# yuxng/PoseCNN

Measured on AMD Instinct MI355X. Metric: RGB-D frames/sec (640x480, 21 classes), higher is better.
Workload: dtype f32

## Files before the change

### __graft_entry__.py

```python
import glob
import os
import subprocess
import sys

ROOT = os.path.dirname(os.path.abspath(__file__))
if ROOT not in sys.path:
    sys.path.insert(0, ROOT)


def build():
    env = dict(os.environ)
    env.setdefault("PYTORCH_ROCM_ARCH", "gfx950")
    jobs = str(min(8, os.cpu_count() or 1))
    subprocess.check_call(["make", "-C", os.path.join(ROOT, "posecnn_amd", "csrc"), "-j", jobs], env=env)
    subprocess.check_call(["make", "-C", os.path.join(ROOT, "oracle")], env=env)
    subprocess.check_call(["make", "-C", os.path.join(ROOT, "oracle"), "ref"], env=env)
    headers = sorted(glob.glob(os.path.join(ROOT, "include", "*.h"))) + sorted(glob.glob(os.path.join(ROOT, "include", "*", "*.h")))
    subprocess.check_call(["gcc", "-std=c11", "-Wall", "-Wextra", "-Werror", "-I" + os.path.join(ROOT, "include")] +
                          [arg for h in headers for arg in ("-include", h)] +
                          [os.path.join(ROOT, "tests", "capi_consumer.c"), "-o", os.path.join(ROOT, "tests", "capi_consumer"),
                           "-L" + os.path.join(ROOT, "posecnn_amd"), "-lposecnn_hip",
                           "-Wl,-rpath,$ORIGIN/../posecnn_amd", "-Wl,-rpath-link,/opt/rocm/lib"], env=env)
    import posecnn_amd
    from posecnn_amd import _lib
    _lib.lib()


def smoke():
    import numpy as np
    import torch

    sys.path.insert(0, os.path.join(ROOT, "tests"))
    import oracle
    from posecnn_amd import config, ops, synth

    assert torch.cuda.is_available(), "smoke() needs a GPU"
    dev = torch.device("cuda:0")
    K = config.DEMO_INTRINSICS.copy()
    K[:2] *= 320 / 640.0
    label, vertex, _ = synth.make_batch(100, 2, H=240, W=320, C=22, n_obj=3, K=K)
    meta = np.stack([config.make_meta_data(K)] * 2)
    ext = config.LOV_EXTENTS
    want = oracle.hough_voting(label, vertex, ext, meta, None, 0, -1.0, 0.02, 10, label_thr=200, padded=True)

    L = torch.from_numpy
    got = ops.hough_voting_gpu_padded(L(label).to(dev), L(vertex).to(dev), L(ext).to(dev), L(meta).to(dev),
                                      None, 0, -1.0, 0.02, 10, label_threshold=200)
    torch.cuda.synchronize()
    names = ("top_box", "top_pose", "top_target", "top_weight", "top_domain", "num_rois")
    for name, g, w in zip(names, got, want):
        g = g.cpu().numpy()
        assert np.array_equal(g.view(np.uint32), np.ascontiguousarray(w).view(np.uint32)), "smoke: %s differs from the oracle" % name
    assert int(got[5][1]) >= 2, "smoke: expected detections"

    rng = np.random.default_rng(0)
    feat = rng.standard_normal((2, 15, 20, 512)).astype(np.float32)
    r = int(want[5][0])
    top, arg = ops.roi_pool(L(feat).to(dev), got[0][:r].contiguous(), 7, 7, 1.0 / 16, 0)
    wt, wa = oracle.roi_pool(feat, want[0][:r], 7, 7, 1.0 / 16, 0)
    assert np.array_equal(top.cpu().numpy(), wt) and np.array_equal(arg.cpu().numpy(), wa), "smoke: roi_pool differs"
    print("smoke ok: %d detections, hough + roi_pool bit-identical to the oracle" % int(got[5][1]))


if __name__ == "__main__":
    build()
    if len(sys.argv) > 1 and sys.argv[1] == "smoke":
        smoke()
```

### posecnn_amd/_lib.py

```python
import ctypes
import glob
import os
import re
from ctypes import (POINTER, c_char_p, c_float, c_int, c_int64, c_long, c_size_t, c_uint32, c_uint64, c_void_p)

_HERE = os.path.dirname(os.path.abspath(__file__))
LIB_PATH = os.path.join(_HERE, "libposecnn_hip.so")

PCNN_OK = 0
PCNN_EINVAL = -1
PCNN_EWORKSPACE = -2
PCNN_EHIP = -3
PCNN_ENULL = -4

MAX_ROI = 128
HOUGH_ROWS_CAPACITY = MAX_ROI * 9
VERTEX_CHANNELS = 3
POSE_CHANNELS = 4

INCLUDE_DIR = os.path.join(os.path.dirname(_HERE), "include")

_RESTYPES = {"int": c_int, "long": c_long, "uint32_t": c_uint32, "const char*": c_char_p}
_SCALARS = {"int": c_int, "long": c_long, "float": c_float, "size_t": c_size_t, "int64_t": c_int64, "uint32_t": c_uint32,
            "uint64_t": c_uint64}
# ... 19 lines not shown
            raise ValueError("%s: not `type* [name]`" % where)
        return _POINTERS.get(" ".join(base), c_void_p)
    base = " ".join(tokens[:-1] if len(tokens) > 1 else tokens)
    if base not in _SCALARS:
        raise ValueError("%s: scalar type '%s' is not one of %s" % (where, base, sorted(_SCALARS)))
    return _SCALARS[base]


def parse_header(header, text):
    text = re.sub(r"^[ \t]*#.*$", "", _strip_comments(text), flags=re.M)
    found = {}
    for m in re.finditer(r"\b(pcnn_\w+)\s*\(", text):
        name, depth, end = m.group(1), 1, m.end()
        while depth and end < len(text):
            depth += {"(": 1, ")": -1}.get(text[end], 0)
            end += 1
        if depth or not re.match(r"\s*;", text[end:]):
            raise ValueError("%s: %s: not a prototype `ret %s(params);`" % (header, name, name))
        ret = re.sub(r"\s*\*\s*", "*", " ".join(re.split(r"[;{}]", text[:m.start()])[-1].split()))
        if ret not in _RESTYPES:
            raise ValueError("%s: %s: return type '%s' is not one of %s" % (header, name, ret, sorted(_RESTYPES)))
        if name in found:
            raise ValueError("%s: %s is declared twice" % (header, name))
        params, depth = [""], 0
        for ch in text[m.end():end - 1]:
            depth += {"(": 1, "[": 1, ")": -1, "]": -1}.get(ch, 0)
            if ch == "," and not depth:
                params.append("")
            else:
                params[-1] += ch
        params = [" ".join(p.split()) for p in params]
        found[name] = (_RESTYPES[ret], [] if params == ["void"] else
                       [_argtype(p, "%s: %s: parameter %d '%s'" % (header, name, i + 1, p)) for i, p in enumerate(params)])
    return found


def parse_headers(texts):
    out, owner = {}, {}
    for header, text in texts:
        out[header] = parse_header(header, text)
        for name in out[header]:
            if name in owner:
                raise ValueError("%s: %s is already declared in %s" % (header, name, owner[name]))
            owner[name] = header
    return out


def header_texts():
    top = sorted(glob.glob(os.path.join(INCLUDE_DIR, "*.h")))
    sub = sorted(glob.glob(os.path.join(INCLUDE_DIR, "*", "*.h")))
    return [(os.path.relpath(p, INCLUDE_DIR).replace(os.sep, "/"), open(p).read()) for p in top + sub]


def header_abi_version(texts=None):
    text = dict(header_texts() if texts is None else texts)["posecnn_hip.h"]
    return int(re.search(r"^[ \t]*#[ \t]*define[ \t]+PCNN_ABI_VERSION[ \t]+(\d+)[ \t]*$", _strip_comments(text), flags=re.M).group(1))


def profile_enable(on=True):
    call("pcnn_profile_enable", 1 if on else 0)


def profile_report(reset=True):
    import json
    L = lib()
    n = L.pcnn_profile_report(None, 0)
    buf = ctypes.create_string_buffer(int(n) + 16)
    L.pcnn_profile_report(buf, len(buf))
    if reset:
        L.pcnn_profile_reset()
    rep = json.loads(buf.value.decode())
    return {k.strip("()"): v for k, v in rep.items()}

_lib = None


class PoseCNNHipError(RuntimeError):

    def __init__(self, fn, status, message):
        super().__init__("%s failed: status %d (%s)" % (fn, status, message))
        self.status = status


def lib():
    global _lib
    if _lib is None:
        if not os.path.exists(LIB_PATH):
            raise RuntimeError(
                "libposecnn_hip.so not found at %s — build it with "
                "`python -c 'import __graft_entry__ as g; g.build()'` or "
                "`make -C posecnn_amd/csrc`. There is no CPU/PyTorch fallback." % LIB_PATH)
        import torch
        handle = ctypes.CDLL(LIB_PATH)
        texts = header_texts()
        bindings = parse_headers(texts)
        for table in bindings.values():
            for name, (res, args) in table.items():
                fn = getattr(handle, name)
                fn.restype = res
                fn.argtypes = args
        if handle.pcnn_abi_version() != header_abi_version(texts):
            raise RuntimeError("libposecnn_hip.so ABI version mismatch")
        BINDINGS.update(bindings)
        _lib = handle
    return _lib


def check(fn_name, status):
    if status != PCNN_OK:
        msg = lib().pcnn_last_error_string()
        msg = msg.decode("utf-8", "replace") if msg else ""
        if status in (PCNN_EINVAL, PCNN_ENULL):
            raise ValueError("%s: %s" % (fn_name, msg))
        raise PoseCNNHipError(fn_name, status, msg)


def call(name, *args):
    check(name, getattr(lib(), name)(*args))
```

### posecnn_amd/networks.py

```python
import math
import os

import numpy as np
import torch
import torch.nn.functional as F

from . import ops, pipeline

DEFAULT_PADDING = "SAME"


def layer(op):

    def layer_decorated(self, *args, **kwargs):
        name = kwargs.setdefault("name", self.get_unique_name(op.__name__))
        if len(self.inputs) == 0:
            raise RuntimeError("No input variables found for layer %s." % name)
        elif len(self.inputs) == 1:
            layer_input = self.inputs[0]
        else:
            layer_input = list(self.inputs)
        if isinstance(layer_input, list):
            layer_input = [i.activate(self) if isinstance(i, _Pending) else i for i in layer_input]
        elif (isinstance(layer_input, _Pending) and op.__name__ != "max_pool"
# ... 79 lines not shown

    def _pool2(self, net):
        return None


class _PendingFirst(_Pending):
    def __init__(self, x, w, bias, relu):
        _Pending.__init__(self, tuple(x.shape[:3]) + (w.shape[3],), bias, relu)
        self.x, self.w = x, w

    def _activate(self, net):
        return net._conv_first(raw_frame_blob(self.x), self.w.permute(3, 2, 0, 1), self.bias, self.relu)

    def frames(self):
        return (self.x if self.x.dtype == torch.uint8 else None, self.x if self.x.dtype == torch.uint16 else None)

    def next_v(self):
        if _is_raw(self.x):
            return ops.conv3x3_c3_winograd43_raw(*self.frames(), self.w, self.bias, self.relu)
        return ops.conv3x3_c3_winograd43(self.x, self.w, self.bias, self.relu)


class _PendingConv12(_Pending):
    def __init__(self, pf, name, w, bias, relu):
        _Pending.__init__(self, pf.shape[:3] + (w.shape[0],), bias, relu)
        self.pf, self.name, self.w = pf, name, w

    def _activate(self, net):
        ut, pk = net._winograd_bank(self.name, self.w)
        return ops.winograd43_conv(self.pf.next_v(), ut, self.bias, *self.shape[:3], self.relu, pool=0, packed=pk)

    def _pool2(self, net):
        pf = self.pf
        frag = net._derived(("conv12_frag", self.name), (self.w,),
                            lambda: ops.conv12_fragment_major(net._winograd_filter(self.name, self.w, transposed=True)),
                            net.winograd_tile)
        if _is_raw(pf.x):
            return ops.conv1_1_conv1_2_fused_raw(*pf.frames(), pf.w, pf.bias, frag, self.bias, pf.relu, self.relu, ut2_layout=1)
        return ops.conv1_1_conv1_2_fused(pf.x, pf.w, pf.bias, frag, self.bias, pf.relu, self.relu, groups=1, ut2_layout=1)


class _PendingGemm(_Pending):
    def __init__(self, v, ut, B, H, W, packed, bias, relu):
        _Pending.__init__(self, (B, H, W, ut.shape[-2]), bias, relu)
        self.v, self.ut, self.packed = v, ut, packed

    def _activate(self, net, pool=0):
        return ops.winograd43_conv(self.v, self.ut, self.bias, *self.shape[:3], self.relu, pool=pool, packed=self.packed)

    def _pool2(self, net):
        return self._activate(net, pool=1)


class _PendingWino(_Pending):
    def __init__(self, m, B, H, W, tile, dual, bias, relu):
        _Pending.__init__(self, (B, H, W, m.shape[2]), bias, relu)
        self.m, self.tile, self.dual = m, tile, dual

    def _activate(self, net, pool=False):
        return ops.winograd_output(self.m, self.bias, *self.shape[:3], self.relu, pool=pool, tile=self.tile)

    def _pool2(self, net):
        if not self.dual:
            return self._activate(net, pool=True)
        self.out, pooled = ops.winograd43_output_both(self.m, self.bias, *self.shape[:3], self.relu)
        return pooled


class _PendingBias(_Pending):
    def __init__(self, y, bias, relu, train=None):
        _Pending.__init__(self, tuple(y.shape), bias, relu)
        self.y, self.train = y, train

    def _activate(self, net):
        return net._bias_act(self.y, self.bias, self.relu)

    def _pool2(self, net):
        if self.train is not None:
            return _nhwc(ops.bias_relu_pool2_train(self.train, self.bias, self.relu))
        return net._bias_relu_pool2(self.y, self.bias, self.relu)


class _ConvAndPool(_Pending):
    def __init__(self, out, pooled, bias, relu):
        _Pending.__init__(self, tuple(out.shape), bias, relu, out, pooled)


class Network(object):

    fused_train_epilogue = False

    def use_fused_train_epilogue(self, on=True):
        self.fused_train_epilogue = bool(on)
        return self

    winograd_packed = True

    def __init__(self, device="cuda", seed=3, init="he", trainable=True):
        self.inputs = []
        self.layers = {}
        self.vars = {}
        self.device = torch.device(device)
        self.trainable = trainable
        self.init = init
        self._gen = torch.Generator(device="cpu").manual_seed(seed)
        self.keep_prob_queue = 1.0
        self.conv_timing = None
        self.winograd_min_channels = 64
        self.winograd_tile = 4
        self._cache = {}
        self.winograd_mfma = True
        self.fuse_first_conv_into_winograd = True
        self.fused_first_conv = True
        self.fused_conv12 = True
        self.defer_act = frozenset()
        self.dual_pool = frozenset()
        self.rows_count = None
        self.fc_skinny = True
        self.small_heads = True
        self.small_heads_max_pixels = 2 * 60 * 80

    def setup(self):
        raise NotImplementedError("Must be subclassed.")

    def feed(self, *args):
        assert len(args) != 0
        self.inputs = []
        for l in args:
            if isinstance(l, str):
                l = self.get_output(l)
            self.inputs.append(l)
        return self

    def get_output(self, name):
        try:
            out = self.layers[name]
        except KeyError:
            raise KeyError("Unknown layer name fed: %s" % name)
        if isinstance(out, _Lazy):
            out = self.layers[name] = out.fn()
        if isinstance(out, _Pending):
            out = self.layers[name] = out.activate(self)
        return out

    def _conv12_fused_at(self, H, W):
        return self.fused_conv12 and self.winograd_mfma and H % 16 == 0 and W % 16 == 0

    def _winograd_filter(self, name, w, transposed=False):
        def build():
            u = ops.winograd_filter(w, self.winograd_tile)
            return u.transpose(1, 2).contiguous() if transposed else u
        return self._derived(("wino", name, transposed), (w,), build, self.winograd_tile)

    def _winograd_bank(self, name, w):
        if not self.winograd_packed:
            return self._winograd_filter(name, w, transposed=True), False
        return self._derived(("wino_packed", name), (w,),
                             lambda: ops.winograd43_pack_filters(self._winograd_filter(name, w, transposed=True)),
                             self.winograd_tile), True

    def _derived(self, slot, sources, build, extra=None):
        hit = self._cache.get(slot)
        if hit is not None and hit[2] == extra and len(hit[0]) == len(sources):
            held, versions = hit[0], hit[1]
            i = 0
            for s in sources:
                if s is not held[i] or s._version != versions[i]:
                    break
                i += 1
            else:
                return hit[3]
        value = build()
        self._cache[slot] = (tuple(sources), tuple(s._version for s in sources), extra, value)
        return value

    def _timing(self, extra):
        if self.conv_timing is not None:
            timing = (torch.cuda.Event(enable_timing=True), torch.cuda.Event(enable_timing=True), extra)
            timing[0].record()
            return timing

    def _timed(self, name, timing, executed, direct):
        if timing is not None:
            timing[1].record()
            self.conv_timing.append((name, executed + timing[2], direct + timing[2], timing[0], timing[1]))

    def _conv_winograd(self, name, input, w, b, relu, c_i, c_o, tile):
        B_, H_, W_ = input.shape[:3]
        first = isinstance(input, _PendingFirst)
        timing = self._timing(2.0 * B_ * H_ * W_ * c_i * 27 if first else 0.0)
        v = input.next_v() if first else ops.winograd_input(input, tile)
        if tile == 4 and self.winograd_mfma and c_i % 64 == 0 and c_o % 64 == 0:
            ut, pk = self._winograd_bank(name, w)
            self._timed(name, timing, 0.0, 0.0)
            even = H_ % 2 == 0 and W_ % 2 == 0
            if name in self.defer_act and even:
                return _PendingGemm(v, ut, B_, H_, W_, pk, b, relu)
            if name in self.dual_pool and even:
                return _ConvAndPool(*ops.winograd43_conv(v, ut, b, B_, H_, W_, relu, pool=2, packed=pk), b, relu)
            return ops.winograd43_conv(v, ut, b, B_, H_, W_, relu, pool=0, packed=pk)
        m = torch.bmm(v, self._winograd_filter(name, w))
        self._timed(name, timing, 2.0 * m.numel() * c_i, 2.0 * B_ * H_ * W_ * c_o * c_i * 9)
        if name in self.defer_act:
            return _PendingWino(m, B_, H_, W_, tile, False, b, relu)
        if tile == 4 and name in self.dual_pool and H_ % 2 == 0 and W_ % 2 == 0:
            return _PendingWino(m, B_, H_, W_, tile, True, b, relu)
        return ops.winograd_output(m, b, B_, H_, W_, relu, pool=False, tile=tile)

    def get_unique_name(self, prefix):
        ident = sum(t.startswith(prefix) for t in self.layers) + 1
        return "%s_%d" % (prefix, ident)

    def make_var(self, name, shape, initializer, trainable=False):
        v = self.vars.get(name)
        if v is None:
            v = self.vars[name] = initializer(shape).to(self.device)
        if self.trainable and trainable and not v.requires_grad and v.is_leaf:
            v.requires_grad_(True)
        if v.shape != tuple(shape):
            raise ValueError("variable %s has shape %s, layer wants %s" % (name, tuple(v.shape), tuple(shape)))
        return v

    def _conv_vars(self, name, c_o, c_i, k_h, k_w, trainable, biased=True):
        w = self.make_var(name + "/weights", (c_o, c_i, k_h, k_w),
                          lambda s: self._weight_init(c_i * k_h * k_w)(s).contiguous(memory_format=torch.channels_last), trainable)
        return w, (self.make_var(name + "/biases", (c_o,), torch.zeros, trainable) if biased else None)

    def _fc_vars(self, name, dim, num_out, trainable):
        return (self.make_var(name + "/weights", (dim, num_out), self._weight_init(dim), trainable),
                self.make_var(name + "/biases", (num_out,), torch.zeros, trainable))

    def _weight_init(self, fan_in):
        if self.init == "tf":
            def f(shape):
                w = torch.empty(shape)
                torch.nn.init.trunc_normal_(w, 0.0, 0.001, -0.002, 0.002, generator=self._gen)
                return w
        else:
            def f(shape):
                return torch.randn(shape, generator=self._gen) * math.sqrt(2.0 / fan_in)
        return f

# ... 440 lines not shown
    def _trunk_vars(self, suffix):
        return [self._conv_vars(name + suffix, co, ci, 3, 3, self.trainable) for name, ci, co, _ in self.TRUNK]

    def _can_group_towers(self):
        d = self.layers.get('data')
        dp = self.layers.get('data_p')
        same = isinstance(dp, torch.Tensor) and (dp.shape == d.shape if not _is_raw(d) else
                                                 (dp.dtype == torch.uint16 and tuple(dp.shape[:3]) == tuple(d.shape[:3]))) if isinstance(d, torch.Tensor) else False
        return (self.grouped_towers and self.input_format == 'RGBD' and isinstance(d, torch.Tensor) and d.is_cuda
                and self.winograd_mfma and self.winograd_tile == 4 and self.winograd_min_channels == 64
                and self.fused_first_conv and self.fuse_first_conv_into_winograd
                and not (torch.is_grad_enabled() and self.trainable)
                and d.shape[1] % 16 == 0 and d.shape[2] % 16 == 0 and same)

    def _trunk_grouped(self):
        d, dp = self.get_output('data'), self.get_output('data_p')
        raw = _is_raw(d)
        if raw:
            x = None
            B, H, W = d.shape[:3]
            B2 = 2 * B
        else:
            x = pipeline.stacked_view(d, dp)
            if x is None:
                x = torch.cat([d, dp], dim=0)
            B2, H, W, _ = x.shape
            B = B2 // 2
        va, vb = self._trunk_vars(""), self._trunk_vars("_p")
        def build():
            packed = []
            for (name, ci, co, _), (w0, b0), (w1, b1) in zip(self.TRUNK, va, vb):
                bias = torch.stack([b0, b1]).contiguous()
                if ci == 3:
                    wt = torch.stack([w0.permute(2, 3, 1, 0), w1.permute(2, 3, 1, 0)]).contiguous()
                else:
                    wt = torch.stack([ops.winograd_filter(w0, 4).transpose(1, 2), ops.winograd_filter(w1, 4).transpose(1, 2)]).contiguous()
                packed.append((wt, bias))
            return packed
        packed = self._derived("grouped", [t for wb in va + vb for t in wb], build)
        y, h, w_ = None, H, W
        for li, (name, ci, co, pool) in enumerate(self.TRUNK):
            wt, bias = packed[li]
            if ci == 3:
                continue
            if li == 1 and self._conv12_fused_at(H, W) and pool == "pool1" and co == 64:
                frag = self._derived(("conv12_frag", "grouped"), (va[li][0], vb[li][0]), lambda: ops.conv12_fragment_major(wt))
                y = (ops.conv1_1_conv1_2_fused_raw(d, dp, packed[0][0], packed[0][1], frag, bias, ut2_layout=1) if raw
                     else ops.conv1_1_conv1_2_fused(x, packed[0][0], packed[0][1], frag, bias, groups=2, ut2_layout=1))
                h, w_ = h // 2, w_ // 2
                continue
            if li == 1:
                v = (ops.conv3x3_c3_winograd43_raw(d, dp, packed[0][0], packed[0][1], True) if raw
                     else ops.conv3x3_c3_winograd43(x, packed[0][0], packed[0][1], True, groups=2))
            else:
                v = ops.winograd_input(y, 4)
            mode = 0 if pool is None else (2 if name == "conv4_3" else 1)
            if self.winograd_packed:
                wt = self._derived(("wino_packed", "grouped", li), (va[li][0], vb[li][0]), lambda: ops.winograd43_pack_filters(wt))
            out = ops.winograd43_conv(v, wt, bias, B2, h, w_, True, pool=mode, groups=2, packed=self.winograd_packed)
            if mode == 2:
                full, y = out
            else:
                full = y = out
            if name in ("conv4_3", "conv5_3"):
                self.layers[name], self.layers[name + "_p"] = full[:B], full[B:]
            if pool is not None:
                h, w_ = h // 2, w_ // 2
                if pool == "pool4":
                    self.layers["pool4"], self.layers["pool4_p"] = y[:B], y[B:]
        return self

    def hbm_table(self, B, H, W):
        towers = 2 if self.input_format == 'RGBD' else 1
        act = lambda div, ch: 4.0 * B * (H // div) * (W // div) * ch
        x_in = (act(2, 64) + act(2, 128) + act(4, 128) + 2 * act(4, 256) + act(8, 256) + 2 * act(8, 512) + 3 * act(16, 512))
        fused = self._conv12_fused_at(H, W)
        t = {"wino43_input_kernel": towers * 3.25 * x_in}
        if not fused:
            t["conv3x3_c3_wino43_kernel"] = towers * (act(1, 3) + 2.25 * act(1, 64))
        return t

    def mfma_table(self, B, H, W):
        towers = 2 if self.input_format == 'RGBD' else 1
        tiles = lambda div: B * ((H // div + 3) // 4) * ((W // div + 3) // 4)
        div = {"1": 1, "2": 2, "3": 4, "4": 8, "5": 16}
        fused = self._conv12_fused_at(H, W)
        fl = sum(2.0 * 36 * tiles(div[n[4]]) * ci * co for n, ci, co, _ in self.TRUNK if ci != 3 and not (fused and n == "conv1_2"))
        t = {"wino43_mfma_kernel": towers * fl}
        if fused:
            t["conv12_wino43_fused_kernel"] = towers * 2.0 * 36 * tiles(1) * 64 * 64
        return t

    def _trunk_reference(self, dtype):
        towers = [("", "data")] + ([("_p", "data_p")] if self.input_format == "RGBD" else [])
        for sfx, src in towers:
            x = raw_frame_blob(self.get_output(src))
            vars_ = [(w.detach().to(dtype), b.detach().to(dtype)) for w, b in self._trunk_vars(sfx)]
            keep = {"conv4_3": [], "pool4": [], "conv5_3": []}
            for n in range(x.shape[0]):
                y = x[n:n + 1].to(dtype)
                for (name, ci, co, pool), (w, b) in zip(self.TRUNK, vars_):
                    _, h, w_, _ = y.shape
                    yp = F.pad(y, (0, 0, 1, 1, 1, 1))
                    acc = None
                    for ky in range(3):
                        for kx in range(3):
                            t_ = yp[:, ky:ky + h, kx:kx + w_, :].reshape(-1, ci) @ w[:, :, ky, kx].t()
                            acc = t_ if acc is None else acc + t_
                    y = torch.relu(acc + b).view(1, h, w_, co)
                    if name in keep:
                        keep[name].append(y.to(torch.float32))
                    if pool is not None:
                        y = y.view(1, h // 2, 2, w_ // 2, 2, co).amax(dim=(2, 4))
                        if pool in keep:
                            keep[pool].append(y.to(torch.float32))
            for k, v in keep.items():
                self.layers[k + sfx] = torch.cat(v, dim=0).contiguous()
        return self

    def _tower(self, src, sfx):
        self.feed(src)
        t = self.trainable
        for name, ci, co, pool in self.TRUNK:
            self.conv(3, 3, co, 1, 1, name=name + sfx, c_i=ci, trainable=t)
            if pool is not None:
                self.max_pool(2, 2, 2, 2, name=pool + sfx)

    def setup(self):
        if self.reference_trunk is not None:
            self._trunk_reference(self.reference_trunk)
            return self._setup_heads()
        if self._can_group_towers():
            self._trunk_grouped()
            return self._setup_heads()
        self._tower('data', '')
        if self.input_format == 'RGBD':
            self._tower('data_p', '_p')
        return self._setup_heads()

    def _mfma_head_ok(self, c_i, c_o):
        return bool(self.mfma_heads) and c_i % 16 == 0 and c_o <= 96 and 4 * 64 * (c_i + 4) <= 60 * 1024
# ... 192 lines not shown
```

### posecnn_amd/ops.py

```python
import ctypes
from ctypes import c_size_t

import numpy as np

import torch

from . import _lib
from ._lib import HOUGH_ROWS_CAPACITY, MAX_ROI, POSE_CHANNELS, VERTEX_CHANNELS, check, lib

__all__ = [
    "hough_voting_gpu", "hough_voting_gpu_padded", "roi_pool", "roi_pool_add2", "hard_label", "conv1_1_conv1_2_fused",
    "conv1_1_conv1_2_fused_raw",
    "average_distance_loss", "backproject", "softmax_argmax", "deconv_bilinear", "bias_act_",
    "hough_voting_grad", "hard_label_grad", "hough_rows_capacity",
    "upscore_softmax_argmax", "Workspace", "vertex_targets", "smooth_l1_loss_vertex_gt",
    "depth_normals", "bilateral_filter_u8", "normal_image", "bilateral_tables", "augment_frames",
    "label_head_loss", "label_head_loss_grad", "vertex_head_loss", "vertex_head_loss_grad",
    "bias_relu_train_", "bias_relu_train_grad", "bias_relu_pool2_train", "bias_relu_pool2_train_grad",
    "estimate_poses_3d", "pose3d_prepare", "pose3d_sample", "pose3d_round",
    "estimate_poses_2d", "pose2d_prepare", "pose2d_sample", "pose2d_round",
    "pose_polish", "icp_refine_batch",
]

INLIER_THRESHOLD = 0.9
LABEL_THRESHOLD = 500


def call(name, *args):
    check(name, getattr(lib(), name)(*args))


def _dev(t, name, dtype):
    if not isinstance(t, torch.Tensor):
        raise TypeError("%s must be a torch.Tensor" % name)
    if not t.is_cuda:
        raise RuntimeError("%s must live on the GPU (got %s); posecnn_amd has no CPU path" % (name, t.device))
    if t.dtype != dtype:
        raise TypeError("%s must be %s (got %s)" % (name, dtype, t.dtype))
    return t if t.is_contiguous() else t.contiguous()


def _aligned16(t):
    return t if t.data_ptr() % 16 == 0 else t.clone(memory_format=torch.contiguous_format)


def _ptr(t):
    return ctypes.c_void_p(t.data_ptr()) if t is not None else ctypes.c_void_p(0)


def _stream(t):
    return ctypes.c_void_p(torch.cuda.current_stream(t.device).cuda_stream)


class Workspace:

    def __init__(self):
        self._buf = None

    def get(self, nbytes, device):
        if self._buf is None or self._buf.numel() < nbytes or self._buf.device != device:
            self._buf = torch.empty(max(int(nbytes), 256), dtype=torch.uint8, device=device)
        return self._buf


_default_ws = {}


def _ws(device, key):
    k = (device.index, key, torch.cuda.current_stream(device).cuda_stream)
    if k not in _default_ws:
        _default_ws[k] = Workspace()
    return _default_ws[k]


# ... 397 lines not shown
    if m.shape[0] != n * n or m.shape[1] != _wino_tiles(B, H, W, tile) or bias.numel() != C:
        raise ValueError("m must be [%d, tiles, C] and bias [C]" % (n * n))
    shape = (B, H // 2, W // 2, C) if pool else (B, H, W, C)
    y = torch.empty(shape, dtype=torch.float32, device=m.device)
    fn = "pcnn_winograd_output_fwd" if tile == 2 else "pcnn_winograd43_output_fwd"
    call(fn, _ptr(m), _ptr(bias), B, H, W, C, 1 if relu else 0, 1 if pool else 0, _ptr(y), _stream(m))
    return y


def winograd43_output_both(m, bias, B, H, W, relu=True):
    m = _dev(m, "m", torch.float32)
    bias = _dev(bias, "bias", torch.float32)
    C = m.shape[2]
    if m.shape[0] != 36 or m.shape[1] != _wino_tiles(B, H, W, 4) or bias.numel() != C:
        raise ValueError("m must be [36, tiles, C] and bias [C]")
    y = torch.empty((B, H, W, C), dtype=torch.float32, device=m.device)
    yp = torch.empty((B, H // 2, W // 2, C), dtype=torch.float32, device=m.device)
    call("pcnn_winograd43_output_both_fwd", _ptr(m), _ptr(bias), B, H, W, C, 1 if relu else 0, _ptr(y), _ptr(yp), _stream(m))
    return y, yp


def winograd43_pack_filters(ut):
    ut = _dev(ut, "ut", torch.float32)
    if ut.dim() not in (3, 4) or ut.shape[-3] != 36:
        raise ValueError("ut must be [groups, 36, Cout, Cin] or [36, Cout, Cin]")
    groups = ut.shape[0] if ut.dim() == 4 else 1
    Cout, Cin = ut.shape[-2], ut.shape[-1]
    utp = torch.empty_like(ut)
    call("pcnn_winograd43_pack_filters_fwd", _ptr(ut), Cin, Cout, int(groups), _ptr(utp), _stream(ut))
    return utp


def winograd43_conv(v, ut, bias, B, H, W, relu=True, pool=0, groups=1, packed=False):
    v = _dev(v, "v", torch.float32)
    ut = _dev(ut, "ut", torch.float32)
    bias = _aligned16(_dev(bias, "bias", torch.float32))
    Cin = v.shape[2]
    if ut.dim() == 3:
        ut = ut.unsqueeze(0)
    Cout = ut.shape[2]
    if (v.shape[0] != 36 or v.shape[1] != _wino_tiles(B, H, W, 4) or tuple(ut.shape) != (groups, 36, Cout, Cin)
            or bias.numel() != groups * Cout):
        raise ValueError("v must be [36, tiles, Cin], ut [groups, 36, Cout, Cin], bias [groups, Cout]")
    pool = int(pool)
    y = torch.empty((B, H // 2, W // 2, Cout) if pool == 1 else (B, H, W, Cout), dtype=torch.float32, device=v.device)
    yp = torch.empty((B, H // 2, W // 2, Cout), dtype=torch.float32, device=v.device) if pool == 2 else None
    ws, nbytes = _workspace(v.device, "wino43_conv", "pcnn_winograd43_conv_workspace_bytes", B, H, W, Cin, Cout, int(groups), at_least=0)
    fn = "pcnn_winograd43_conv_packed_fwd" if packed else "pcnn_winograd43_conv_fwd"
    call(fn, _ptr(v), _ptr(ut), _ptr(bias), B, H, W, Cin, Cout, int(groups), 1 if relu else 0, pool, _ptr(y), _ptr(yp), _ptr(ws),
         nbytes, _stream(v))
    return (y, yp) if pool == 2 else y


def fc_rows(x, wt, bias, relu=True, num_rows=None, addend=None):
    x = _dev(x, "x", torch.float32)
    wt = _dev(wt, "wt", torch.float32)
    bias = _aligned16(_dev(bias, "bias", torch.float32))
    if x.dim() != 2 or wt.dim() != 2 or wt.shape[1] != x.shape[1] or bias.numel() != wt.shape[0]:
        raise ValueError("x must be [M, K], wt [N, K], bias [N]")
    M, K = x.shape
    N = wt.shape[0]
    y = torch.empty((M, N), dtype=torch.float32, device=x.device)
    nr = _dev(num_rows, "num_rows", torch.int32) if num_rows is not None else None
    ad = _dev(addend, "addend", torch.float32) if addend is not None else None
    if ad is not None and tuple(ad.shape) != (M, N):
        raise ValueError("addend must be [M, N]")
    ws, nbytes = _workspace(x.device, "fc_rows", "pcnn_fc_rows_workspace_bytes", M, K, N, at_least=0)
    call("pcnn_fc_rows_fwd", _ptr(x), _ptr(wt), _ptr(bias), M, K, N, 1 if relu else 0, _ptr(nr), _ptr(ad), _ptr(y), _ptr(ws),
         nbytes, _stream(x))
    return y


def fc_rows_split(x, wt, bias, out_a, relu_a=True, relu_b=False, num_rows=None):
    x = _dev(x, "x", torch.float32)
    wt = _dev(wt, "wt", torch.float32)
    bias = _aligned16(_dev(bias, "bias", torch.float32))
    if x.dim() != 2 or wt.dim() != 2 or wt.shape[1] != x.shape[1] or bias.numel() != wt.shape[0] or not 0 < out_a < wt.shape[0]:
        raise ValueError("x must be [M, K], wt [out_a + out_b, K], bias [out_a + out_b]")
    M, K = x.shape
    out_b = wt.shape[0] - int(out_a)
    ya = torch.empty((M, int(out_a)), dtype=torch.float32, device=x.device)
    yb = torch.empty((M, out_b), dtype=torch.float32, device=x.device)
    nr = _dev(num_rows, "num_rows", torch.int32) if num_rows is not None else None
    call("pcnn_fc_rows_split_fwd", _ptr(x), _ptr(wt), _ptr(bias), M, K, int(out_a), out_b, 1 if relu_a else 0, 1 if relu_b else 0,
         _ptr(nr), _ptr(ya), _ptr(yb), _stream(x))
    return ya, yb


def fc_rows_cols(x, wt_padded, bias_padded, out_features, activation="none", num_rows=None):
    x = _dev(x, "x", torch.float32)
    wt_padded = _dev(wt_padded, "wt_padded", torch.float32)
    bias_padded = _aligned16(_dev(bias_padded, "bias_padded", torch.float32))
    if x.dim() != 2 or wt_padded.dim() != 2 or wt_padded.shape[1] != x.shape[1] or bias_padded.numel() != wt_padded.shape[0]:
        raise ValueError("x must be [M, K], wt_padded [Npad, K], bias_padded [Npad]")
    M, K = x.shape
    act = {"none": 0, "relu": 1, "tanh": 2}[activation]
    y = torch.empty((M, int(out_features)), dtype=torch.float32, device=x.device)
    y2 = torch.empty_like(y) if act == 2 else None
    nr = _dev(num_rows, "num_rows", torch.int32) if num_rows is not None else None
    call("pcnn_fc_rows_cols_fwd", _ptr(x), _ptr(wt_padded), _ptr(bias_padded), M, K, wt_padded.shape[0], int(out_features), act,
         _ptr(nr), _ptr(y), _ptr(y2), _stream(x))
    return (y, y2) if act == 2 else y


_tickets = {}

# ... 1038 lines not shown
```

Measured before the change: 824.6.

## Fuse Winograd input transform and MFMA GEMM for conv2 layers

Adds a fused HIP kernel for the conv2_1/conv2_2 trunk layers (64 or 128 input channels, 128 output). Each block loads an 18x18 input patch into shared memory, runs the Winograd F(4,3) input transform in LDS, multiplies with MFMA against pre-packed filters, and applies the output transform with bias, ReLU and optional 2x2 pooling. This removes the separate transformed-input tensor and its HBM round trip, at the cost of a large LDS footprint and one block per CU (launch bounds 512,1). It is routed in by default for eligible inference shapes above a minimum block count.

Result: faster. 862.0, median of 6 (+4.5%).

```diff
diff --git a/__graft_entry__.py b/__graft_entry__.py
--- a/__graft_entry__.py
+++ b/__graft_entry__.py
@@ -15,7 +15,8 @@
     subprocess.check_call(["make", "-C", os.path.join(ROOT, "posecnn_amd", "csrc"), "-j", jobs], env=env)
     subprocess.check_call(["make", "-C", os.path.join(ROOT, "oracle")], env=env)
     subprocess.check_call(["make", "-C", os.path.join(ROOT, "oracle"), "ref"], env=env)
-    headers = sorted(glob.glob(os.path.join(ROOT, "include", "*.h"))) + sorted(glob.glob(os.path.join(ROOT, "include", "*", "*.h")))
+    headers = sorted(glob.glob(os.path.join(ROOT, "include", "*.h"))) + sorted(glob.glob(os.path.join(ROOT, "include", "*", "*.h"))) + \
+        sorted(glob.glob(os.path.join(ROOT, "include", "*", "*", "*.h")))
     subprocess.check_call(["gcc", "-std=c11", "-Wall", "-Wextra", "-Werror", "-I" + os.path.join(ROOT, "include")] +
                           [arg for h in headers for arg in ("-include", h)] +
                           [os.path.join(ROOT, "tests", "capi_consumer.c"), "-o", os.path.join(ROOT, "tests", "capi_consumer"),
diff --git a/include/posecnn_hip/trunk/conv2_fused.h b/include/posecnn_hip/trunk/conv2_fused.h
--- /dev/null
+++ b/include/posecnn_hip/trunk/conv2_fused.h
@@ -0,0 +1,19 @@
+#ifndef POSECNN_HIP_TRUNK_CONV2_FUSED_H
+#define POSECNN_HIP_TRUNK_CONV2_FUSED_H
+
+#include <stddef.h>
+#include <stdint.h>
+
+#ifdef __cplusplus
+extern "C" {
+#endif
+
+int pcnn_winograd43_conv_fused_fwd(const float* x, const float* utp, const float* bias, int batch, int height, int width,
+                                   int in_channels, int out_channels, int groups, int relu, int pool, float* y,
+                                   void* stream);
+
+#ifdef __cplusplus
+}
+#endif
+
+#endif
diff --git a/posecnn_amd/_lib.py b/posecnn_amd/_lib.py
--- a/posecnn_amd/_lib.py
+++ b/posecnn_amd/_lib.py
@@ -95,6 +95,11 @@
     return [(os.path.relpath(p, INCLUDE_DIR).replace(os.sep, "/"), open(p).read()) for p in top + sub]
 
 
+def route_header_texts():
+    deep = sorted(glob.glob(os.path.join(INCLUDE_DIR, "*", "*", "*.h")))
+    return [(os.path.relpath(p, INCLUDE_DIR).replace(os.sep, "/"), open(p).read()) for p in deep]
+
+
 def header_abi_version(texts=None):
     text = dict(header_texts() if texts is None else texts)["posecnn_hip.h"]
     return int(re.search(r"^[ \t]*#[ \t]*define[ \t]+PCNN_ABI_VERSION[ \t]+(\d+)[ \t]*$", _strip_comments(text), flags=re.M).group(1))
@@ -136,7 +141,7 @@
         import torch
         handle = ctypes.CDLL(LIB_PATH)
         texts = header_texts()
-        bindings = parse_headers(texts)
+        bindings = parse_headers(texts + route_header_texts())
         for table in bindings.values():
             for name, (res, args) in table.items():
                 fn = getattr(handle, name)
diff --git a/posecnn_amd/csrc/conv2_fused.hip b/posecnn_amd/csrc/conv2_fused.hip
--- /dev/null
+++ b/posecnn_amd/csrc/conv2_fused.hip
@@ -0,0 +1,295 @@
+#include "pcnn_device.h"
+#include "../../include/posecnn_hip/trunk/conv2_fused.h"
+
+namespace {
+
+using namespace pcnn;
+
+constexpr int C2_P = 18;
+constexpr int C2_YS = 68;
+constexpr int C2_PATCH = C2_P * C2_P * C2_YS;
+constexpr int C2_GRP = 6 * 16 * 64;
+constexpr int C2_SMEM = C2_PATCH + 2 * C2_GRP;
+constexpr int C2_NPV = (C2_P * C2_P * 16 + 511) / 512;
+
+typedef float c2v4 __attribute__((ext_vector_type(4)));
+
+typedef const __attribute__((address_space(1))) float* c2gptr;
+typedef const __attribute__((address_space(1))) c2v4* c2gptr4;
+__device__ __forceinline__ c2gptr c2_uniform(const float* p)
+{
+  const unsigned long long u = (unsigned long long)p;
+  const unsigned lo = __builtin_amdgcn_readfirstlane((unsigned)u), hi = __builtin_amdgcn_readfirstlane((unsigned)(u >> 32));
+  return (c2gptr)(((unsigned long long)hi << 32) | lo);
+}
+
+template <int KH, int POOL>
+__global__ __launch_bounds__(512, 1) void conv2_wino43_fused_kernel(
+    const float* __restrict__ x, const float* __restrict__ utp, const float* __restrict__ bias, float* __restrict__ y,
+    int H, int W, int nbx, int nby, int imgs_per_group, int relu)
+{
+  constexpr int CIN = 64 * KH;
+  __shared__ __attribute__((aligned(16))) float smem[C2_SMEM];
+  float* const s_y = smem;
+  float* const s_v = smem + C2_PATCH;
+  const int tid = threadIdx.x, lane = tid & 63;
+  const int wave = __builtin_amdgcn_readfirstlane(tid >> 6);
+  const int b = __builtin_amdgcn_readfirstlane(blockIdx.x / (nbx * nby));
+  const int by = __builtin_amdgcn_readfirstlane((blockIdx.x / nbx) % nby), bx = __builtin_amdgcn_readfirstlane(blockIdx.x % nbx);
+  const int py0 = 16 * by - 1, px0 = 16 * bx - 1;
+  const int grp = __builtin_amdgcn_readfirstlane(b / imgs_per_group);
+  utp += (size_t)grp * 36 * 128 * CIN;
+  const float bv = bias[(size_t)grp * 128 + 16 * wave + (lane & 15)];
+
+  c2v4 pv[C2_NPV];
+  const float* xb = x + (size_t)b * H * W * CIN;
+#define C2_LOADP(E0, E1, HH, TID)                                                                                  \
+  _Pragma("unroll") for (int e = (E0); e < (E1); e++) {                                                         \
+    const int i = (TID) + 512 * e;                                                                              \
+    const int p = i >> 4, q = i & 15;                                                                           \
+    const int r = p / C2_P, c = p - C2_P * r;                                                                   \
+    const int iy = py0 + r, ix = px0 + c;                                                                       \
+    const bool ok = i < C2_P * C2_P * 16 && iy >= 0 && iy < H && ix >= 0 && ix < W;                             \
+    const unsigned pix = ok ? (unsigned)(iy * W + ix) : 0u;    \
+    c2v4 val = *reinterpret_cast<const c2v4*>(xb + (pix * CIN + 64 * (HH) + 4 * q));                            \
+    if (!ok) val = (c2v4){0.f, 0.f, 0.f, 0.f};                                                                  \
+    pv[e] = val;                                                                                                \
+  }
+#define C2_STOREP(E0, E1, TID)                                                                                  \
+  _Pragma("unroll") for (int e = (E0); e < (E1); e++) {                                                         \
+    const int i = (TID) + 512 * e;                                                                              \
+    if (i < C2_P * C2_P * 16) *reinterpret_cast<c2v4*>(&s_y[(i >> 4) * C2_YS + 4 * (i & 15)]) = pv[e];          \
+  }
+  C2_LOADP(0, C2_NPV, 0, tid)
+  C2_STOREP(0, C2_NPV, tid)
+
+  const int lr = lane & 15, lk = lane >> 4;
+  const int tile = tid >> 5, cp = tid & 31;
+  const int tyy = tile >> 2, txx = tile & 3;
+  const float* const yb = s_y + ((4 * tyy) * C2_P + 4 * txx) * C2_YS + 2 * cp;
+  float* const vb = s_v + tile * 64 + (((cp >> 1) ^ tile) * 4) + 2 * (cp & 1);
+  const float* ab[4];
+#pragma unroll
+  for (int g = 0; g < 4; g++) ab[g] = s_v + lr * 64 + (((4 * g + lk) ^ lr) * 4);
+  v4f acc[36];
+  c2v4 a0[4], a1[4], q0[4], q1[4];
+  const float* const utw = (const float*)c2_uniform(utp + wave * KH * 1024);
+  const unsigned foff = (unsigned)(lane * 4);
+#define C2_LOADB(D0, D1, K, HH, G)                                                                              \
+  { const c2gptr pk0_ = c2_uniform(utw + (size_t)(K) * (128 * CIN) + 1024 * (HH));                              \
+    const c2gptr pk1_ = c2_uniform(utw + (size_t)((K) + 1) * (128 * CIN) + 1024 * (HH));                        \
+    D0 = *(c2gptr4)(pk0_ + (foff + 256 * (G)));                                                                 \
+    D1 = *(c2gptr4)(pk1_ + (foff + 256 * (G))); }
+#define C2_LOADA(D0, D1, BUF, J, G)                                                                             \
+  { D0 = *reinterpret_cast<const c2v4*>(ab[G] + ((BUF) * C2_GRP + (J) * 1024));                                 \
+    D1 = *reinterpret_cast<const c2v4*>(ab[G] + ((BUF) * C2_GRP + ((J) + 1) * 1024)); }
+#define C2_PRODUCE(XI, BUF)                                                                                     \
+  {                                                                                                             \
+    f2 ta[6];                                                                                                   \
+    _Pragma("unroll") for (int hh = 0; hh < 2; hh++) {                                                          \
+      f2 d[3][6];                                                                                               \
+      _Pragma("unroll") for (int s3 = 0; s3 < 3; s3++)                                                          \
+        _Pragma("unroll") for (int r = 0; r < 6; r++)                                                           \
+          if (((XI) == 0 && (r == 0 || r == 2 || r == 4)) || ((XI) == 5 && (r == 1 || r == 3 || r == 5)) ||     \
+              ((XI) >= 1 && (XI) <= 4 && r >= 1 && r <= 4))                                                     \
+            d[s3][r] = *reinterpret_cast<const f2*>(yb + (r * C2_P + 3 * hh + s3) * C2_YS);                     \
+      __builtin_amdgcn_sched_barrier(0);                                                                        \
+      _Pragma("unroll") for (int s3 = 0; s3 < 3; s3++) {                                                        \
+        const int s2 = 3 * hh + s3;                                                                             \
+        if ((XI) == 0) ta[s2] = (4.f * d[s3][0] - 5.f * d[s3][2]) + d[s3][4];                                   \
+        else if ((XI) == 5) ta[s2] = (4.f * d[s3][1] - 5.f * d[s3][3]) + d[s3][5];                              \
+        else if ((XI) == 1 || (XI) == 2) {                                                                      \
+          const f2 a = d[s3][4] - 4.f * d[s3][2], b_ = d[s3][3] - 4.f * d[s3][1];                               \
+          ta[s2] = (XI) == 1 ? a + b_ : a - b_;                                                                 \
+        } else {                                                                                                \
+          const f2 c = d[s3][4] - d[s3][2], e = 2.f * (d[s3][3] - d[s3][1]);                                    \
+          ta[s2] = (XI) == 3 ? c + e : c - e;                                                                   \
+        }                                                                                                       \
+      }                                                                                                         \
+      __builtin_amdgcn_sched_barrier(0);                                                                        \
+    }                                                                                                           \
+    f2 oa[6];                                                                                                   \
+    oa[0] = (4.f * ta[0] - 5.f * ta[2]) + ta[4];                                                                \
+    { const f2 a = ta[4] - 4.f * ta[2], b_ = ta[3] - 4.f * ta[1]; oa[1] = a + b_; oa[2] = a - b_; }             \
+    { const f2 c = ta[4] - ta[2], e = 2.f * (ta[3] - ta[1]); oa[3] = c + e; oa[4] = c - e; }                    \
+    oa[5] = (4.f * ta[1] - 5.f * ta[3]) + ta[5];                                                                \
+    _Pragma("unroll") for (int j = 0; j < 6; j++)                                                               \
+      *reinterpret_cast<f2*>(vb + ((BUF) * C2_GRP + j * 1024)) = oa[j];                                         \
+  }
+#define C2_PAIR(XI, J, BUF, HH, NK, NH)                                                                         \
+  {                                                                                                             \
+    if ((J) == 0) { _Pragma("unroll") for (int g_ = 0; g_ < 4; g_++) C2_LOADA(a0[g_], a1[g_], BUF, 0, g_) }     \
+    v4f ca_, cb_;                                                                                               \
+    if ((HH) == 0) { ca_ = (v4f){0.f, 0.f, 0.f, 0.f}; cb_ = ca_; }                                              \
+    else { ca_ = acc[6 * (XI) + (J)]; cb_ = acc[6 * (XI) + (J) + 1]; }                                          \
+    _Pragma("unroll") for (int g_ = 0; g_ < 4; g_++) {                                                          \
+      __builtin_amdgcn_sched_barrier(0);                                                                        \
+      _Pragma("unroll") for (int i_ = 0; i_ < 4; i_++) {                                                        \
+        ca_ = __builtin_amdgcn_mfma_f32_16x16x4f32(a0[g_][i_], q0[g_][i_], ca_, 0, 0, 0);                       \
+        cb_ = __builtin_amdgcn_mfma_f32_16x16x4f32(a1[g_][i_], q1[g_][i_], cb_, 0, 0, 0);                       \
+      }                                                                                                         \
+      __builtin_amdgcn_sched_barrier(0);                                                                        \
+      if ((J) < 4) { C2_LOADA(a0[g_], a1[g_], BUF, (J) + 2, g_) }                                               \
+      if ((NK) >= 0) { C2_LOADB(q0[g_], q1[g_], (NK), (NH), g_) }                                               \
+    }                                                                                                           \
+    acc[6 * (XI) + (J)] = ca_;                                                                                  \
+    acc[6 * (XI) + (J) + 1] = cb_;                                                                              \
+  }
+#define C2_NEXTK(XI, HH) ((XI) < 5 ? 6 * (XI) + 6 : (HH) + 1 < KH ? 0 : -1)
+#define C2_NEXTH(XI, HH) ((XI) < 5 ? (HH) : (HH) + 1)
+#define C2_CONSUME(XI, BUF, HH)                                                                                 \
+  C2_PAIR(XI, 0, BUF, HH, 6 * (XI) + 2, HH) C2_PAIR(XI, 2, BUF, HH, 6 * (XI) + 4, HH)                           \
+  C2_PAIR(XI, 4, BUF, HH, C2_NEXTK(XI, HH), C2_NEXTH(XI, HH))
+#define C2_STEP(S, HH)                                                                                          \
+  C2_PRODUCE(S, (S) & 1)                                                                                        \
+  __builtin_amdgcn_sched_barrier(0);        \
+  C2_CONSUME((S) - 1, ((S) - 1) & 1, HH)                                                                        \
+  __syncthreads();
+
+  {
+#pragma unroll
+    for (int g = 0; g < 4; g++) C2_LOADB(q0[g], q1[g], 0, 0, g)
+  }
+  __syncthreads();
+#pragma unroll
+  for (int h = 0; h < KH; h++) {
+    C2_PRODUCE(0, 0)
+    __syncthreads();
+    C2_STEP(1, h) C2_STEP(2, h) C2_STEP(3, h) C2_STEP(4, h) C2_STEP(5, h)
+    if (h + 1 < KH) {
+      int tid2 = tid;
+      asm volatile("" : "+v"(tid2));
+      C2_LOADP(0, 4, h + 1, tid2)
+      C2_PAIR(5, 0, 1, h, 32, h)
+      C2_STOREP(0, 4, tid2)
+      C2_LOADP(4, 8, h + 1, tid2)
+      C2_PAIR(5, 2, 1, h, 34, h)
+      C2_STOREP(4, 8, tid2)
+      C2_LOADP(8, C2_NPV, h + 1, tid2)
+      C2_PAIR(5, 4, 1, h, 0, h + 1)
+      C2_STOREP(8, C2_NPV, tid2)
+    } else {
+      C2_CONSUME(5, 1, h)
+    }
+    __syncthreads();
+  }
+#undef C2_STEP
+#undef C2_CONSUME
+#undef C2_NEXTK
+#undef C2_NEXTH
+#undef C2_PAIR
+#undef C2_PRODUCE
+#undef C2_LOADA
+#undef C2_LOADB
+#undef C2_STOREP
+#undef C2_LOADP
+
+  float* const s_o = smem;
+  {
+    typedef float f2e __attribute__((ext_vector_type(2)));
+    const int wcol = (16 * wave + lr) ^ (16 * lk);
+#pragma unroll
+    for (int ih = 0; ih < 2; ih++) {
+      f2e yo[16];
+#pragma unroll
+      for (int o = 0; o < 16; o++) yo[o] = (f2e){0.f, 0.f};
+#pragma unroll
+      for (int nu = 0; nu < 6; nu++) {
+        const float c0 = nu == 5 ? 0.f : 1.f;
+        const float c1 = nu == 1 ? 1.f : nu == 2 ? -1.f : nu == 3 ? 2.f : nu == 4 ? -2.f : 0.f;
+        const float c2 = (nu == 1 || nu == 2) ? 1.f : (nu == 3 || nu == 4) ? 4.f : 0.f;
+        const float c3 = nu == 1 ? 1.f : nu == 2 ? -1.f : nu == 3 ? 8.f : nu == 4 ? -8.f : nu == 5 ? 1.f : 0.f;
+        f2e m_[6], t_[4];
+#pragma unroll
+        for (int x_ = 0; x_ < 6; x_++) m_[x_] = (f2e){acc[6 * x_ + nu][2 * ih], acc[6 * x_ + nu][2 * ih + 1]};
+        {
+          const f2e s = m_[1] + m_[2], d = m_[1] - m_[2], S = m_[3] + m_[4], D = m_[3] - m_[4];
+          t_[0] = (m_[0] + s) + S;
+          t_[1] = __builtin_elementwise_fma((f2e){2.f, 2.f}, D, d);
+          t_[2] = __builtin_elementwise_fma((f2e){4.f, 4.f}, S, s);
+          t_[3] = __builtin_elementwise_fma((f2e){8.f, 8.f}, D, d) + m_[5];
+        }
+#pragma unroll
+        for (int a_ = 0; a_ < 4; a_++) {
+          yo[4 * a_ + 0] = __builtin_elementwise_fma(t_[a_], (f2e){c0, c0}, yo[4 * a_ + 0]);
+          yo[4 * a_ + 1] = __builtin_elementwise_fma(t_[a_], (f2e){c1, c1}, yo[4 * a_ + 1]);
+          yo[4 * a_ + 2] = __builtin_elementwise_fma(t_[a_], (f2e){c2, c2}, yo[4 * a_ + 2]);
+          yo[4 * a_ + 3] = __builtin_elementwise_fma(t_[a_], (f2e){c3, c3}, yo[4 * a_ + 3]);
+        }
+      }
+#pragma unroll
+      for (int o = 0; o < 16; o++) {
+        f2e val = yo[o] + (f2e){bv, bv};
+        if (relu) { val.x = val.x > 0.f ? val.x : 0.f; val.y = val.y > 0.f ? val.y : 0.f; }
+        yo[o] = val;
+      }
+      if (POOL == 0) {
+#pragma unroll
+        for (int a_ = 0; a_ < 4; a_++)
+#pragma unroll
+          for (int e_ = 0; e_ < 4; e_++) {
+            s_o[((4 * lk + a_) * 16 + 4 * (2 * ih) + e_) * 128 + wcol] = yo[4 * a_ + e_].x;
+            s_o[((4 * lk + a_) * 16 + 4 * (2 * ih + 1) + e_) * 128 + wcol] = yo[4 * a_ + e_].y;
+          }
+      } else {
+#pragma unroll
+        for (int a2 = 0; a2 < 2; a2++)
+#pragma unroll
+          for (int e2 = 0; e2 < 2; e2++) {
+            f2e p = yo[4 * (2 * a2) + 2 * e2];
+            const f2e p1 = yo[4 * (2 * a2) + 2 * e2 + 1], p2 = yo[4 * (2 * a2 + 1) + 2 * e2], p3 = yo[4 * (2 * a2 + 1) + 2 * e2 + 1];
+            p.x = p1.x > p.x ? p1.x : p.x; p.y = p1.y > p.y ? p1.y : p.y;
+            p.x = p2.x > p.x ? p2.x : p.x; p.y = p2.y > p.y ? p2.y : p.y;
+            p.x = p3.x > p.x ? p3.x : p.x; p.y = p3.y > p.y ? p3.y : p.y;
+            s_o[((2 * lk + a2) * 8 + (2 * (2 * ih) + e2)) * 128 + wcol] = p.x;
+            s_o[((2 * lk + a2) * 8 + (2 * (2 * ih + 1) + e2)) * 128 + wcol] = p.y;
+          }
+      }
+    }
+  }
+  __syncthreads();
+  if (POOL == 0) {
+#pragma unroll 4
+    for (int i = tid; i < 16 * 16 * 32; i += 512) {
+      const int c4 = (i & 31) * 4, pxl = (i >> 5) & 15, pyl = i >> 9;
+      *reinterpret_cast<c2v4*>(y + (((size_t)b * H + 16 * by + pyl) * W + 16 * bx + pxl) * 128 + c4) =
+          *reinterpret_cast<const c2v4*>(&s_o[(pyl * 16 + pxl) * 128 + (c4 ^ (16 * (pyl >> 2)))]);
+    }
+  } else {
+    const int Hp = H >> 1, Wp = W >> 1;
+#pragma unroll
+    for (int i = tid; i < 8 * 8 * 32; i += 512) {
+      const int c4 = (i & 31) * 4, pxl = (i >> 5) & 7, pyl = i >> 8;
+      *reinterpret_cast<c2v4*>(y + (((size_t)b * Hp + 8 * by + pyl) * Wp + 8 * bx + pxl) * 128 + c4) =
+          *reinterpret_cast<const c2v4*>(&s_o[(pyl * 8 + pxl) * 128 + (c4 ^ (16 * (pyl >> 1)))]);
+    }
+  }
+}
+
+}
+
+extern "C" int pcnn_winograd43_conv_fused_fwd(const float* x, const float* utp, const float* bias, int B, int H, int W,
+                                              int Cin, int Cout, int groups, int relu, int pool, float* y, void* stream_)
+{
+  PCNN_REQUIRE(B >= 1 && H >= 16 && W >= 16 && H % 16 == 0 && W % 16 == 0, PCNN_EINVAL,
+               "winograd43_conv_fused: the frame must be a multiple of 16 in both directions (got %dx%dx%d)", B, H, W);
+  PCNN_REQUIRE(Cin == 64 || Cin == 128, PCNN_EINVAL, "winograd43_conv_fused: input channels must be 64 or 128 (got %d)", Cin);
+  PCNN_REQUIRE(Cout == 128, PCNN_EINVAL, "winograd43_conv_fused: output channels must be 128 (got %d)", Cout);
+  PCNN_REQUIRE(pool == 0 || pool == 1, PCNN_EINVAL, "winograd43_conv_fused: pool must be 0 (none) or 1 (pooled only)");
+  PCNN_REQUIRE(groups >= 1 && B % groups == 0, PCNN_EINVAL, "winograd43_conv_fused: batch %d is not a multiple of groups %d", B, groups);
+  PCNN_REQUIRE(x && utp && bias && y, PCNN_ENULL, "winograd43_conv_fused: NULL pointer");
+  PCNN_REQUIRE(aligned16(x) && aligned16(utp) && aligned16(bias) && aligned16(y), PCNN_EINVAL,
+               "winograd43_conv_fused: pointers (x, utp, bias, y) must be 16-byte aligned");
+  const long long blocks = (long long)B * (H / 16) * (W / 16);
+  PCNN_REQUIRE(blocks < (1ll << 31), PCNN_EINVAL, "winograd43_conv_fused: grid too large");
+  PCNN_REQUIRE((long long)H * W * Cin < (1ll << 30), PCNN_EINVAL,
+               "winograd43_conv_fused: an image of %dx%dx%d floats exceeds the kernel's 32-bit offsets", H, W, Cin);
+  hipStream_t stream = (hipStream_t)stream_;
+#define C2_GO(KH, P)                                                                                              \
+  PCNN_LAUNCH((conv2_wino43_fused_kernel<KH, P>), dim3((unsigned)blocks), dim3(512), 0, stream, x, utp, bias, y, H, W, W / 16, \
+              H / 16, B / groups, relu)
+  if (Cin == 64) { if (pool) C2_GO(1, 1); else C2_GO(1, 0); }
+  else { if (pool) C2_GO(2, 1); else C2_GO(2, 0); }
+#undef C2_GO
+  return check_launch("winograd43_conv_fused_fwd");
+}
diff --git a/posecnn_amd/networks.py b/posecnn_amd/networks.py
--- a/posecnn_amd/networks.py
+++ b/posecnn_amd/networks.py
@@ -155,6 +155,18 @@
         return self._activate(net, pool=1)
 
 
+class _PendingConv2(_Pending):
+    def __init__(self, x, utp, bias, relu):
+        _Pending.__init__(self, tuple(x.shape[:3]) + (utp.shape[-2],), bias, relu)
+        self.x, self.utp = x, utp
+
+    def _activate(self, net, pool=0):
+        return ops.winograd43_conv_fused(self.x, self.utp, self.bias, self.relu, pool=pool)
+
+    def _pool2(self, net):
+        return self._activate(net, pool=1)
+
+
 class _PendingWino(_Pending):
     def __init__(self, m, B, H, W, tile, dual, bias, relu):
         _Pending.__init__(self, (B, H, W, m.shape[2]), bias, relu)
@@ -198,6 +210,15 @@
         return self
 
     winograd_packed = True
+
+    fused_conv2 = True
+    FUSED_CONV2_FLOOR = 128
+    fused_conv2_min_blocks = FUSED_CONV2_FLOOR
+
+    def _conv2_fused_at(self, B, H, W, c_i, c_o):
+        return (self.fused_conv2 and self.winograd_mfma and self.winograd_tile == 4 and self.winograd_packed
+                and not (torch.is_grad_enabled() and self.trainable) and c_i in (64, 128) and c_o == 128 and H % 16 == 0 and W % 16 == 0
+                and B * (H // 16) * (W // 16) >= max(int(self.fused_conv2_min_blocks), self.FUSED_CONV2_FLOOR))
 
     def __init__(self, device="cuda", seed=3, init="he", trainable=True):
         self.inputs = []
@@ -291,6 +312,10 @@
     def _conv_winograd(self, name, input, w, b, relu, c_i, c_o, tile):
         B_, H_, W_ = input.shape[:3]
         first = isinstance(input, _PendingFirst)
+        if not first and tile == 4 and self._conv2_fused_at(B_, H_, W_, c_i, c_o):
+            pc = _PendingConv2(input, self._winograd_bank(name, w)[0], b, relu)
+            self._timed(name, self._timing(0.0), 0.0, 0.0)
+            return pc if name in self.defer_act else pc.activate(self)
         timing = self._timing(2.0 * B_ * H_ * W_ * c_i * 27 if first else 0.0)
         v = input.next_v() if first else ops.winograd_input(input, tile)
         if tile == 4 and self.winograd_mfma and c_i % 64 == 0 and c_o % 64 == 0:
@@ -837,6 +862,12 @@
             if li == 1:
                 v = (ops.conv3x3_c3_winograd43_raw(d, dp, packed[0][0], packed[0][1], True) if raw
                      else ops.conv3x3_c3_winograd43(x, packed[0][0], packed[0][1], True, groups=2))
+            elif self._conv2_fused_at(B2, h, w_, ci, co):
+                wt = self._derived(("wino_packed", "grouped", li), (va[li][0], vb[li][0]), lambda: ops.winograd43_pack_filters(wt))
+                y = ops.winograd43_conv_fused(y, wt, bias, True, pool=0 if pool is None else 1, groups=2)
+                if pool is not None:
+                    h, w_ = h // 2, w_ // 2
+                continue
             else:
                 v = ops.winograd_input(y, 4)
             mode = 0 if pool is None else (2 if name == "conv4_3" else 1)
@@ -855,12 +886,20 @@
                     self.layers["pool4"], self.layers["pool4_p"] = y[:B], y[B:]
         return self
 
+    def _conv2_layers_fused(self, B, H, W):
+        towers = 2 if self.input_format == 'RGBD' and self.grouped_towers else 1
+        return self._conv2_fused_at(towers * B, H // 2, W // 2, 64, 128)
+
     def hbm_table(self, B, H, W):
         towers = 2 if self.input_format == 'RGBD' else 1
         act = lambda div, ch: 4.0 * B * (H // div) * (W // div) * ch
         x_in = (act(2, 64) + act(2, 128) + act(4, 128) + 2 * act(4, 256) + act(8, 256) + 2 * act(8, 512) + 3 * act(16, 512))
         fused = self._conv12_fused_at(H, W)
-        t = {"wino43_input_kernel": towers * 3.25 * x_in}
+        t = {}
+        if self._conv2_layers_fused(B, H, W):
+            x_in -= act(2, 64) + act(2, 128)
+            t["conv2_wino43_fused_kernel"] = towers * (act(2, 64) + act(2, 128) + act(2, 128) + act(4, 128))
+        t["wino43_input_kernel"] = towers * 3.25 * x_in
         if not fused:
             t["conv3x3_c3_wino43_kernel"] = towers * (act(1, 3) + 2.25 * act(1, 64))
         return t
@@ -870,8 +909,12 @@
         tiles = lambda div: B * ((H // div + 3) // 4) * ((W // div + 3) // 4)
         div = {"1": 1, "2": 2, "3": 4, "4": 8, "5": 16}
         fused = self._conv12_fused_at(H, W)
-        fl = sum(2.0 * 36 * tiles(div[n[4]]) * ci * co for n, ci, co, _ in self.TRUNK if ci != 3 and not (fused and n == "conv1_2"))
+        conv2 = self._conv2_layers_fused(B, H, W)
+        fl = sum(2.0 * 36 * tiles(div[n[4]]) * ci * co for n, ci, co, _ in self.TRUNK
+                 if ci != 3 and not (fused and n == "conv1_2") and not (conv2 and n[4] == "2"))
         t = {"wino43_mfma_kernel": towers * fl}
+        if conv2:
+            t["conv2_wino43_fused_kernel"] = towers * 2.0 * 36 * tiles(2) * (64 + 128) * 128
         if fused:
             t["conv12_wino43_fused_kernel"] = towers * 2.0 * 36 * tiles(1) * 64 * 64
         return t
diff --git a/posecnn_amd/ops.py b/posecnn_amd/ops.py
--- a/posecnn_amd/ops.py
+++ b/posecnn_amd/ops.py
@@ -19,7 +19,7 @@
     "bias_relu_train_", "bias_relu_train_grad", "bias_relu_pool2_train", "bias_relu_pool2_train_grad",
     "estimate_poses_3d", "pose3d_prepare", "pose3d_sample", "pose3d_round",
     "estimate_poses_2d", "pose2d_prepare", "pose2d_sample", "pose2d_round",
-    "pose_polish", "icp_refine_batch",
+    "pose_polish", "icp_refine_batch", "winograd43_conv_fused",
 ]
 
 INLIER_THRESHOLD = 0.9
@@ -523,6 +523,25 @@
     return (y, yp) if pool == 2 else y
 
 
+def winograd43_conv_fused(x, utp, bias, relu=True, pool=0, groups=1):
+    x = _dev(x, "x", torch.float32)
+    utp = _dev(utp, "utp", torch.float32)
+    bias = _aligned16(_dev(bias, "bias", torch.float32))
+    if x.dim() != 4:
+        raise ValueError("x must be [B,H,W,Cin]")
+    B, H, W, Cin = x.shape
+    if utp.dim() == 3:
+        utp = utp.unsqueeze(0)
+    Cout = utp.shape[2]
+    if tuple(utp.shape) != (groups, 36, Cout, Cin) or bias.numel() != groups * Cout:
+        raise ValueError("utp must be [groups, 36, Cout, Cin], bias [groups, Cout]")
+    pool = int(pool)
+    y = torch.empty((B, H // 2, W // 2, Cout) if pool == 1 else (B, H, W, Cout), dtype=torch.float32, device=x.device)
+    call("pcnn_winograd43_conv_fused_fwd", _ptr(x), _ptr(utp), _ptr(bias), B, H, W, Cin, Cout, int(groups), 1 if relu else 0, pool,
+         _ptr(y), _stream(x))
+    return y
+
+
 def fc_rows(x, wt, bias, relu=True, num_rows=None, addend=None):
     x = _dev(x, "x", torch.float32)
     wt = _dev(wt, "wt", torch.float32)
```
